# musyoku/chainer-speech-recognition

Hardware: AMD Instinct MI355X
Metric: utterances/sec (T=1000, 40x3 feat, |V|~3000) CTC train step (higher is better)
Workload: dtype bf16

## Files before the change

chainer-speech-recognition_amd/asr/_lib.py:

```python
import ctypes
import os

import torch

_HERE = os.path.dirname(os.path.abspath(__file__))
_ACT = os.environ.get("ASR_ACT", "").lower()
LIB_PATH = os.environ.get("ASR_HIP_LIB") or os.path.join(os.path.dirname(_HERE),
                                                        "libasr_hip_f16.so" if _ACT in ("f16", "fp16", "float16", "half") else "libasr_hip.so")

_lib = None


def act_dtype():
    return torch.float16 if lib().asr_act_dtype() else torch.bfloat16


def debug_flag(key, default):
    for item in os.environ.get("ASR_DEBUG", "").split(","):
        k, _, v = item.strip().partition("=")
        if k == key and v:
            return int(v)
    return default

c_void_p, c_int, c_float, c_size_t = ctypes.c_void_p, ctypes.c_int, ctypes.c_float, ctypes.c_size_t
# ... 150 lines not shown
    "asr_crelu_bwd": (c_int, [c_void_p] * 4 + [c_longlong, c_int]),
    "asr_softmax_fwd": (c_int, [c_void_p] * 3 + [c_longlong, c_int, c_int]),
    "asr_softmax_bwd": (c_int, [c_void_p] * 4 + [c_longlong, c_int, c_int]),
    "asr_avgpool_h_fwd": (c_int, [c_void_p] * 3 + [c_longlong, c_int, c_int, c_int]),
    "asr_avgpool_h_bwd": (c_int, [c_void_p] * 3 + [c_longlong, c_int, c_int, c_int]),
    "asr_unpool_h_fwd": (c_int, [c_void_p] * 3 + [c_longlong, c_int, c_int, c_int, c_int]),
    "asr_unpool_h_bwd": (c_int, [c_void_p] * 3 + [c_longlong, c_int, c_int, c_int, c_int]),
    "asr_gaussian_noise": (c_int, [c_void_p] * 3 + [c_longlong, c_float, ctypes.c_uint]),
    "asr_maxpool_h_indexes": (c_int, [c_void_p, c_void_p, c_void_p, c_longlong, c_int, c_int, c_int]),
    "asr_upsample_h_fwd": (c_int, [c_void_p] * 4 + [c_longlong] + [c_int] * 4),
    "asr_upsample_h_bwd": (c_int, [c_void_p] * 4 + [c_longlong] + [c_int] * 4),
    "asr_spp_bins": (c_int, [c_int]),
    "asr_spp_fwd": (c_int, [c_void_p] * 4 + [c_int] * 5),
    "asr_spp_bwd": (c_int, [c_void_p] * 4 + [c_int] * 5),
    "asr_sgd_ctl": (c_int, [c_void_p] * 4 + [c_longlong, c_int] + [c_float] * 3 + [c_void_p]),
}

_ERRORS = {-1: "bad argument", -2: "workspace too small", -3: "unsupported shape", -4: "kernel launch failed"}


class AsrHipError(RuntimeError):
    pass


def lib():
    global _lib
    if _lib is None:
        if not os.path.isfile(LIB_PATH):
            raise AsrHipError("%s not found: build it with `make -C %s` (hipcc, gfx950). There is no CPU fallback."
                              % (LIB_PATH, os.path.dirname(LIB_PATH)))
# ... 27 lines not shown
```

chainer-speech-recognition_amd/asr/_ops.py:

```python
import os

import torch

from . import _lib
from ._lib import check, ptr, stream

BF16 = _lib.act_dtype()
F32 = torch.float32


def _is_bf16(t):
    if t.dtype == BF16:
        return 1
    if t.dtype == F32:
        return 0
    raise TypeError("expected float32 or bfloat16, got %s" % t.dtype)


def gemm_nt(a, b, bias=None, out_dtype=BF16, out=None):
    assert a.dtype == BF16 and b.dtype == BF16 and a.dim() == 2 and b.dim() == 2
    assert a.stride(1) == 1 and b.stride(1) == 1 and a.shape[1] == b.shape[1]
    M, K = a.shape
    N = b.shape[0]
    if out is None:
# ... 528 lines not shown
def clear_abort_words(dev):
    for w in abort_words():
        if w.device == dev:
            w.zero_()


def step_control(g, partials, clip, grad_scale, alpha, beta1, beta2, applied, ctl, any_abort=None, reserved_index=-1, loss_scale=None):
    if any_abort is None:
        any_abort = gather_abort(g.device)
    rc = _lib.lib().asr_step_control_scaled(stream(), ptr(g), g.numel(), ptr(partials), ptr(any_abort), None, float(clip),
                                            float(grad_scale), float(alpha), float(beta1), float(beta2), ptr(applied), ptr(ctl),
                                            int(reserved_index), None if loss_scale is None else ptr(loss_scale))
    check(rc, "asr_step_control_scaled")


def sqnorm_partials_count(n):
    return int(_lib.lib().asr_sqnorm_partials_count(int(n)))


def adam_ctl(p, g, m, v, beta1, beta2, eps, weight_decay, ctl):
    rc = _lib.lib().asr_adam_ctl(stream(), ptr(p), ptr(g), ptr(m), ptr(v), p.numel(), beta1, beta2, eps, weight_decay, ptr(ctl))
    check(rc, "asr_adam_ctl")


def sgd_ctl(p, g, v, kind, lr, momentum, weight_decay, ctl):
    rc = _lib.lib().asr_sgd_ctl(stream(), ptr(p), ptr(g), ptr(v), p.numel(), int(kind), lr, momentum, weight_decay, ptr(ctl))
    check(rc, "asr_sgd_ctl")


SRU_CHUNKED = [True]
# ... 568 lines not shown
```

chainer-speech-recognition_amd/asr/functions.py:

```python
import math
import os

import torch

from . import _ops
from ._lib import debug_flag as _lib_debug
from .link import grad_buffer, grads_queued

BF16, F32 = _ops.BF16, torch.float32


_SIDE = {"streams": {}, "origins": {}, "enabled": True, "dirty": set(), "keep": [], "keep_bytes": 0,
         "join_before_recurrence": _lib_debug("side_join", 0) != 0}
_KEEP_LIMIT = 512
_KEEP_BYTES_LIMIT = int(_lib_debug("side_keep_gb", 48)) << 30


def side_stream():
    if not _SIDE["enabled"]:
        return None
    cur = torch.cuda.current_stream()
    key = cur.cuda_stream
    st = _SIDE["streams"].get(key)
    if st is None:
# ... 359 lines not shown


def conv_weight_matrix_bwd(W):
    return _ops.conv_weight_pack_bwd(W.contiguous())


def conv_weight_matrix_pad8(W):
    Co, Ci, KH, KW = W.shape
    Wp = torch.zeros((Co, 8, KH, KW), dtype=W.dtype, device=W.device)
    Wp[:, :Ci] = W
    return _ops.conv_weight_pack(Wp, Kp=(KH * KW * 8 + 31) // 32 * 32)


def convolution_2d(x, W, b, link, pad=(0, 0), causal=False, out_f32=False):
    pad_h, pad_t = (pad, pad) if isinstance(pad, int) else pad
    w16 = link.compute_copy("w16", W, conv_weight_matrix)
    w16t = link.compute_copy("w16t", W, conv_weight_matrix_t)
    wbwd = link.compute_copy("wbwd", W, conv_weight_matrix_bwd) if _ops.conv_implicit_ok(W.shape[0], W.shape[2], W.shape[3]) else None
    if x.dtype not in (F32, BF16):
        raise TypeError("convolution input must be float32 or bfloat16")
    w16p = link.compute_copy("w16p", W, conv_weight_matrix_pad8) if W.shape[1] < 8 else None
    y = _Conv2D.apply(x, W, b, w16, w16t, wbwd, w16p, int(pad_h), int(pad_t), bool(causal), bool(out_f32))
    return logical4(y)


def convolution_2d_given_weight(x, W, b, link, pad=(0, 0), causal=False, out_f32=False):
    pad_h, pad_t = (pad, pad) if isinstance(pad, int) else pad
    with torch.no_grad():
        w16 = conv_weight_matrix(W.detach())
        w16t = conv_weight_matrix_t(W.detach())
        wbwd = conv_weight_matrix_bwd(W.detach()) if _ops.conv_implicit_ok(W.shape[0], W.shape[2], W.shape[3]) else None
        w16p = conv_weight_matrix_pad8(W.detach()) if W.shape[1] < 8 else None
    y = _Conv2D.apply(x, W, b, w16, w16t, wbwd, w16p, int(pad_h), int(pad_t), bool(causal), bool(out_f32))
    return logical4(y)


# ... 51 lines not shown
        return False
    Co, Ci, KH, KW = wshape
    if not _ops.conv_mp_ok(Ci, KH, KW, Co, k) or Ci >= 8:
        return False
    return x.shape[2] + 2 * pad_h - KH + 1 >= 1 and (x.shape[3] if causal else x.shape[3] + 2 * pad_t - KW + 1) >= 1


def convolution_maxout_pool(x, W, b, link, pad, causal, k, given_weight=False):
    pad_h, pad_t = (pad, pad) if isinstance(pad, int) else pad
    if not convolution_maxout_pool_ok(x, tuple(W.shape), pad, causal, k):
        return None
    if given_weight:
        with torch.no_grad():
            w16q = conv_weight_matrix_pad8_128(W.detach())
    else:
        w16q = link.compute_copy("w16q", W, conv_weight_matrix_pad8_128)
    return logical4(_ConvMaxoutPool.apply(x, W, b, w16q, int(pad_h), int(pad_t), bool(causal), int(k)))


class _Dense(torch.autograd.Function):

    @staticmethod
    def forward(ctx, x2, W, b, w16, w16t, out_f32):
        y = _ops.gemm_nt(x2, w16, b.detach() if b is not None else None, F32 if out_f32 else BF16)
        ctx.save_for_backward(x2, w16t)
        ctx.params = (W, b)
        ctx.need_dx = ctx.needs_input_grad[0]
        if out_f32:
            ctx._asr_mailbox = _GradMailbox(y, b)
        return y

# ... 686 lines not shown
```

chainer-speech-recognition_amd/asr/link.py:

```python
import contextlib
import math

import torch

from . import _lib

F32 = torch.float32
BF16 = _lib.act_dtype()

_WEIGHT_EPOCH = [0]


def bump_weight_epoch():
    _WEIGHT_EPOCH[0] += 1


class Parameter(torch.nn.Parameter):

    def __new__(cls, data=None):
        if data is None:
            data = torch.empty(0, dtype=F32)
        return super().__new__(cls, data, requires_grad=True)


class Link(torch.nn.Module):
    def __init__(self):
        super().__init__()
        object.__setattr__(self, "_compute_cache", {})
        object.__setattr__(self, "_cast_registry", {})

    @contextlib.contextmanager
    def init_scope(self):
        yield

    @property
    def xp(self):
        return torch

    def params(self):
        return self.parameters()

    def namedparams(self):
        for name, p in self.named_parameters():
            yield "/" + name.replace(".", "/"), p
# ... 18 lines not shown
            if p is not None and p.numel() == 0 and src is not None and src.numel() > 0:
                p.data = torch.empty(src.shape, dtype=p.dtype, device=p.device)
        super()._load_from_state_dict(state_dict, prefix, *args, **kwargs)
        bump_weight_epoch()

    def compute_copy(self, key, param, maker, layout=None):
        stamp = (_WEIGHT_EPOCH[0], param._version, param.data_ptr())
        hit = self._compute_cache.get(key)
        if hit is not None and hit[0] == stamp:
            _await_copy(hit)
            return hit[1]
        with torch.no_grad():
            value = maker(param.detach())
        self._compute_cache[key] = _made_copy(stamp, value)
        if layout is not None and value.is_cuda:
            self._cast_registry[key] = (param, value, _cast_jobs(param, layout))
        return value


def _made_copy(stamp, value):
    if not value.is_cuda:
        return (stamp, value, None, None)
    cur = torch.cuda.current_stream()
    return (stamp, value, {"stream": cur, "event": None}, {cur.cuda_stream})


def _await_copy(entry):
    if entry[2] is None:
        return
    cur = torch.cuda.current_stream()
    if cur.cuda_stream not in entry[3]:
# ... 8 lines not shown

def _cast_jobs(param, layout):
    n, shape = param.numel(), tuple(param.shape)
    if layout == "plain":
        return ((0, 0, n // shape[-1], shape[-1], 0),)
    if layout == "t_first":
        return ((0, 0, shape[0], n // shape[0], 1),)
    if layout == "t_last":
        return ((0, 0, n // shape[-1], shape[-1], 1),)
    if layout == "t_each":
        each = shape[-2] * shape[-1]
        return tuple((i * each, i * each, shape[-2], shape[-1], 1) for i in range(n // each))
    raise ValueError(layout)


def refresh_compute_copies(model):
    from . import _lib
    todo, sig = [], []
    for m in model.modules():
        reg = getattr(m, "_cast_registry", None)
        if not reg:
            continue
        for key, (param, out, jobs) in reg.items():
            hit = m._compute_cache.get(key)
            if hit is None or hit[1] is not out or hit[0][2] != param.data_ptr() or not param.is_cuda:
                continue
            todo.append((m, key, param, out))
            sig.append((param.data_ptr(), out.data_ptr(), jobs))
    if not todo:
        return 0
    cached = getattr(model, "_cast_table", None)
    if cached is None or cached[0] != sig:
        rows, tile = [], 0
        for src, dst, jobs in sig:
            for so, do, r, c, t in jobs:
                rows.append([src + 4 * so, dst + 2 * do, r, c, t, tile])
                tile += ((r + 63) // 64) * ((c + 63) // 64)
        table = torch.tensor(rows, dtype=torch.int64).to(todo[0][2].device)
        cached = (sig, table, len(rows), tile)
        object.__setattr__(model, "_cast_table", cached)
    _lib.check(_lib.lib().asr_cast_bf16_many(_lib.stream(), _lib.ptr(cached[1]), cached[2], cached[3]), "asr_cast_bf16_many")
    for m, key, param, out in todo:
        m._compute_cache[key] = _made_copy((_WEIGHT_EPOCH[0], param._version, param.data_ptr()), out)
    return cached[2]


class Chain(Link):
    pass


_GRAD_LISTENER = [None]


def grads_queued(*params):
    if _GRAD_LISTENER[0] is not None:
        _GRAD_LISTENER[0]([p for p in params if p is not None])


def grad_buffer(param):
# ... 89 lines not shown
```

chainer-speech-recognition_amd/asr/optimizers.py:

```python
import torch

from . import _ops
from .link import bump_weight_epoch, refresh_compute_copies

F32 = torch.float32
RESERVED = 64


class GradientClipping(object):
    name = "GradientClipping"

    def __init__(self, threshold):
        self.threshold = threshold


class WeightDecay(object):
    name = "WeightDecay"

    def __init__(self, rate):
        self.rate = rate


class Optimizer(object):
    def __init__(self):
# ... 66 lines not shown
        any_abort = _ops.gather_abort(G.device, G[0:1] if self.communicator is not None else None)
        scale = 1.0
        if self.communicator is not None:
            self.communicator.finish_backward(self)
            scale = 1.0 / self.communicator.size
        self.t += 1
        clip, decay = 0.0, 0.0
        for h in self._hooks:
            if isinstance(h, GradientClipping):
                clip = float(h.threshold)
            elif isinstance(h, WeightDecay):
                decay = float(h.rate)
        alpha, beta1, beta2 = self._control_constants()
        _ops.step_control(G, self._flat["partials"], clip, scale, alpha, beta1, beta2, self._flat["applied"], self._flat["ctl"],
                          any_abort, 0, self._loss_scale_buffer(G.device))
        self._step(P, G, decay, self._flat["ctl"])
        bump_weight_epoch()
        refresh_compute_copies(self.target)
        try:
            self._raise_if_previous_step_gave_up()
        finally:
            self._watch_gave_up()

    def _watch_gave_up(self):
        st = self._gave_up
        if st[0] is None:
            st[0] = torch.zeros(1, dtype=F32).pin_memory()
        if st[1] is None or st[1].query():
            st[0].copy_(self._flat["ctl"][6:7], non_blocking=True)
            st[1] = torch.cuda.Event()
            st[1].record()
            st[2] = self.t

# ... 110 lines not shown
        self.alpha, self.beta1, self.beta2, self.eps = alpha, beta1, beta2, eps

        self.m = self.v = None

    def _init_state(self, total, dev, old):
        self.m = self._carried(total, dev, old, self.m)
        self.v = self._carried(total, dev, old, self.v)

    def _control_constants(self):
        return self.alpha, self.beta1, self.beta2

    def _state_buffers(self):
        return [self.m, self.v]

    def _step(self, P, G, decay, ctl):
        _ops.adam_ctl(P, G, self.m, self.v, self.beta1, self.beta2, self.eps, decay, ctl)


class SGD(Optimizer):
    kind = 0

    def __init__(self, lr=0.01):
        super().__init__()
        self.lr = lr
        self.momentum = 0.0
        self.vel = None

    def _init_state(self, total, dev, old):
        if self.kind:
            self.vel = self._carried(total, dev, old, self.vel)

# ... 75 lines not shown
```

chainer-speech-recognition_amd/csrc/elementwise.hip:

```cpp
#include "common.hpp"
#include "../../include/asr_hip.h"

namespace asr {
namespace ew {

constexpr int kThreads = 256;
static inline int grid_for(long long n) {
    long long g = (n + kThreads - 1) / kThreads;
    if (g > 256 * 16) g = 256 * 16;
    if (g < 1) g = 1;
    return (int)g;
}

__global__ void cast_bf16_kernel(const float* __restrict__ src, uint16_t* __restrict__ dst, long long n) {
    for (long long i = blockIdx.x * (long long)blockDim.x + threadIdx.x; i < n; i += (long long)gridDim.x * blockDim.x)
        dst[i] = f32_to_bf16(src[i]);
}
__global__ void cast_bf16_vec8_kernel(const float4* __restrict__ src, uint4* __restrict__ dst, long long n8) {
    for (long long i = blockIdx.x * (long long)blockDim.x + threadIdx.x; i < n8; i += (long long)gridDim.x * blockDim.x) {
        const float4 a = src[2 * i], b = src[2 * i + 1];
        uint4 o;
        o.x = (uint32_t)f32_to_bf16(a.x) | ((uint32_t)f32_to_bf16(a.y) << 16);
        o.y = (uint32_t)f32_to_bf16(a.z) | ((uint32_t)f32_to_bf16(a.w) << 16);
        o.z = (uint32_t)f32_to_bf16(b.x) | ((uint32_t)f32_to_bf16(b.y) << 16);
// ... 401 lines not shown
        if (transpose) dst[(long long)k * Co + co] = f32_to_bf16(v); else dst[i] = f32_to_bf16(v);
    }
}
__global__ void conv_weight_pack_bwd_kernel(const float* __restrict__ W, uint16_t* __restrict__ dst, int Co, int Ci, int KH,
                                            int KW) {
    const long long n = (long long)Co * Ci * KH * KW;
    for (long long i = blockIdx.x * (long long)blockDim.x + threadIdx.x; i < n; i += (long long)gridDim.x * blockDim.x) {
        long long r = i;
        const int co = (int)(r % Co); r /= Co;
        const int kw = (int)(r % KW); r /= KW;
        const int kh = (int)(r % KH);
        const int ci = (int)(r / KH);
        dst[i] = f32_to_bf16(W[(((long long)co * Ci + ci) * KH + kh) * KW + kw]);
    }
}
__global__ void conv_weight_grad_unpack_kernel(const float* __restrict__ scratch, float* __restrict__ gW, int Co, int Ci,
                                               int KH, int KW, int Kp, int Cs, int copies) {
    const long long n = (long long)Co * Ci * KH * KW;
    for (long long i = blockIdx.x * (long long)blockDim.x + threadIdx.x; i < n; i += (long long)gridDim.x * blockDim.x) {
        long long r = i;
        const int kw = (int)(r % KW); r /= KW;
        const int kh = (int)(r % KH); r /= KH;
        const int ci = (int)(r % Ci);
        const int co = (int)(r / Ci);
        const long long o = (long long)co * Kp + (kh * KW + kw) * Cs + ci;
        float v = scratch[o];
        for (int c = 1; c < copies; ++c) v += scratch[o + (long long)c * Co * Kp];
        gW[i] += v;
    }
}
// ... 567 lines not shown
    if (!x || !y || n <= 0 || ratio < 0.f || ratio >= 1.f) return ASR_ERR_BAD_ARG;
    hipLaunchKernelGGL(dropout_kernel, dim3(grid_for(n)), dim3(kThreads), 0, (hipStream_t)stream, (const uint16_t*)x,
                       (uint16_t*)y, n, ratio, seed);
    ASR_LAUNCH_CHECK();
    return ASR_OK;
}

extern "C" int asr_conv_weight_pack(void* stream, const float* W, void* dst, int Co, int Ci, int KH, int KW, int Kp,
                                    int transpose) {
    if (!W || !dst || Co <= 0 || Ci <= 0 || KH <= 0 || KW <= 0 || Kp < KH * KW * Ci) return ASR_ERR_BAD_ARG;
    hipLaunchKernelGGL(conv_weight_pack_kernel, dim3(grid_for((long long)Co * Kp)), dim3(kThreads), 0, (hipStream_t)stream,
                       W, (uint16_t*)dst, Co, Ci, KH, KW, Kp, transpose);
    ASR_LAUNCH_CHECK();
    return ASR_OK;
}
extern "C" int asr_conv_weight_pack_bwd(void* stream, const float* W, void* dst, int Co, int Ci, int KH, int KW) {
    if (!W || !dst || Co <= 0 || Ci <= 0 || KH <= 0 || KW <= 0) return ASR_ERR_BAD_ARG;
    hipLaunchKernelGGL(conv_weight_pack_bwd_kernel, dim3(grid_for((long long)Co * Ci * KH * KW)), dim3(kThreads), 0, (hipStream_t)stream,
                       W, (uint16_t*)dst, Co, Ci, KH, KW);
    ASR_LAUNCH_CHECK();
    return ASR_OK;
}
extern "C" int asr_conv_weight_grad_unpack_copies(void* stream, const float* scratch, int copies, float* gW, int Co, int Ci, int KH,
                                                  int KW, int Kp, int Cs) {
    if (Cs <= 0) Cs = Ci;
    if (!scratch || !gW || Co <= 0 || Ci <= 0 || KH <= 0 || KW <= 0 || Cs < Ci || Kp < KH * KW * Cs || copies < 1 || copies > 8)
        return ASR_ERR_BAD_ARG;
    hipLaunchKernelGGL(conv_weight_grad_unpack_kernel, dim3(grid_for((long long)Co * Ci * KH * KW)), dim3(kThreads), 0,
                       (hipStream_t)stream, scratch, gW, Co, Ci, KH, KW, Kp, Cs, copies);
    ASR_LAUNCH_CHECK();
// ... 27 lines not shown
```

chainer-speech-recognition_amd/csrc/optim.hip:

```cpp
#include "common.hpp"
#include "../../include/asr_hip.h"

namespace asr {
namespace optim {

__global__ __launch_bounds__(256) void sqnorm_kernel(const float* __restrict__ g, long long n, float* __restrict__ out) {
    __shared__ float scratch[32];
    float s = 0.f;
    for (long long i = blockIdx.x * (long long)blockDim.x + threadIdx.x; i < n; i += (long long)gridDim.x * blockDim.x) {
        const float v = g[i];
        s += v * v;
    }
    s = block_sum(s, scratch);
    if (threadIdx.x == 0) atomicAdd(out, s);
}

__global__ __launch_bounds__(256) void adam_kernel(float* __restrict__ p, const float* __restrict__ g,
                                                   float* __restrict__ m, float* __restrict__ v, long long n, float lr_t,
                                                   float beta1, float beta2, float eps, float decay, float clip,
                                                   float grad_scale, const float* __restrict__ sqnorm) {
    float rate = grad_scale;
    if (sqnorm) {
        if (!isfinite(sqnorm[0])) return;
        if (clip > 0.f) {
// ... 98 lines not shown
        const float r = clip / norm;
        if (r < 1.f) rate *= r;
    }
    int t = applied[0];
    if (!drop) applied[0] = ++t;
    const double tt = t < 1 ? 1.0 : (double)t;
    const double fix1 = 1.0 - pow((double)beta1, tt), fix2 = 1.0 - pow((double)beta2, tt);
    ctl[0] = drop ? 1.f : 0.f;
    ctl[1] = rate;
    ctl[2] = (float)((double)alpha * sqrt(fix2) / fix1);
    ctl[3] = (float)t;
    ctl[5] = gave_up ? 1.f : 0.f;
    if (gave_up) ctl[6] += 1.f;
}

__global__ __launch_bounds__(256) void adam_ctl_kernel(float* __restrict__ p, const float* __restrict__ g, float* __restrict__ m,
                                                       float* __restrict__ v, long long n, float beta1, float beta2, float eps,
                                                       float decay, const float* __restrict__ ctl) {
    if (ctl[0] != 0.f) return;
    const float rate = ctl[1], lr_t = ctl[2];
    for (long long i = blockIdx.x * (long long)blockDim.x + threadIdx.x; i < n; i += (long long)gridDim.x * blockDim.x) {
        const float pi = p[i];
        const float gi = g[i] * rate + decay * pi;
        float mi = m[i], vi = v[i];
        mi += (1.f - beta1) * (gi - mi);
        vi += (1.f - beta2) * (gi * gi - vi);
        m[i] = mi;
        v[i] = vi;
        p[i] = pi - lr_t * mi / (sqrtf(vi) + eps);
    }
}

__global__ __launch_bounds__(256) void sgd_ctl_kernel(float* __restrict__ p, const float* __restrict__ g, float* __restrict__ v,
                                                      long long n, int kind, float lr, float mu, float decay,
                                                      const float* __restrict__ ctl) {
    if (ctl[0] != 0.f) return;
    const float rate = ctl[1];
    for (long long i = blockIdx.x * (long long)blockDim.x + threadIdx.x; i < n; i += (long long)gridDim.x * blockDim.x) {
        const float pi = p[i];
        const float gi = g[i] * rate + decay * pi;
        if (kind == 0) {
            p[i] = pi - lr * gi;
        } else {
            const float vi = mu * v[i] - lr * gi;
// ... 81 lines not shown
                                float clip_threshold, float grad_scale, float alpha, float beta1, float beta2,
                                int* applied_steps, float* ctl, int reserved_index) {
    return asr_step_control_scaled(stream, g, n, partials, abort0, abort1, clip_threshold, grad_scale, alpha, beta1, beta2,
                                   applied_steps, ctl, reserved_index, nullptr);
}

extern "C" int asr_adam_ctl(void* stream, float* p, const float* g, float* m, float* v, long long n, float beta1, float beta2,
                            float eps, float weight_decay, const float* ctl) {
    if (!p || !g || !m || !v || !ctl || n <= 0) return ASR_ERR_BAD_ARG;
    hipLaunchKernelGGL(adam_ctl_kernel, dim3(grid_for(n)), dim3(256), 0, (hipStream_t)stream, p, g, m, v, n, beta1, beta2, eps,
                       weight_decay, ctl);
    ASR_LAUNCH_CHECK();
    return ASR_OK;
}

extern "C" int asr_sgd_ctl(void* stream, float* p, const float* g, float* v, long long n, int kind, float lr, float momentum,
                           float weight_decay, const float* ctl) {
    if (!p || !g || !ctl || n <= 0 || kind < 0 || kind > 2 || (kind > 0 && !v)) return ASR_ERR_BAD_ARG;
    hipLaunchKernelGGL(sgd_ctl_kernel, dim3(grid_for(n)), dim3(256), 0, (hipStream_t)stream, p, g, v, n, kind, lr, momentum,
                       weight_decay, ctl);
    ASR_LAUNCH_CHECK();
    return ASR_OK;
}
```

include/asr_hip.h:

```cpp
#ifndef ASR_HIP_H
#define ASR_HIP_H
#include <stddef.h>
#include <stdint.h>
#ifdef __cplusplus
extern "C" {
#endif

int asr_version(void);
int asr_act_dtype(void);
int asr_stream_delay(void* stream, int microseconds);
int asr_occupy_cus(void* stream, int microseconds, int lds_bytes, int blocks);
int asr_stream_traffic(void* stream, int microseconds, int lds_bytes, int blocks, void* buf, long long bytes);

size_t asr_ctc_workspace_bytes(int T, int B, int V, int Lmax, int gram);
int asr_ctc_forward(void* stream, const float* xs, const int32_t* label_unigram, const int32_t* label_bigram,
                    const int32_t* x_len, const int32_t* l_len, int T, int B, int V, int Lmax, int blank,
                    float* loss_per_utt, float* loss_mean, void* workspace, size_t workspace_bytes);
int asr_ctc_forward_lse(void* stream, const float* xs, const int32_t* label_unigram, const int32_t* label_bigram,
                        const int32_t* x_len, const int32_t* l_len, int T, int B, int V, int Lmax, int blank, float* loss_per_utt,
                        float* loss_mean, void* workspace, size_t workspace_bytes, const float* row_lse);
int asr_ctc_backward(void* stream, const float* xs, const int32_t* x_len, int T, int B, int V, int Lmax, int gram,
                     const float* gy, int gy_per_utt, float scale, float* grad, const void* workspace,
                     size_t workspace_bytes);
int asr_ctc_loss_grad(void* stream, const float* xs, const int32_t* label_unigram, const int32_t* label_bigram,
// ... 126 lines not shown
                       int KH, int KW, int Tr, int Hr, int N);
int asr_conv_nt_8pn(void* stream, const void* x, const void* W, int ldw, void* out, int out_bf16, const float* bias, int Ts, int B, int Hs,
                    int Cs, int KH, int KW, int pad_h, int pad_t, int sgn, int Tr, int Hr, int N);
int asr_conv_direct_ok(int Ts, int B, int Hs, int Cs, int KH, int KW, int Tr, int Hr, int N, int K, int out_bf16);
int asr_conv_direct_nt(void* stream, const void* x, const void* W, int ldw, void* out, const float* bias, int Ts, int B, int Hs, int Cs,
                       int KH, int KW, int pad_h, int pad_t, int sgn, int Tr, int Hr, int N);
int asr_conv_mp_ok(int Ci, int KH, int KW, int Co, int k);
int asr_conv_mp_fwd(void* stream, const void* x8, const void* W, int ldw, const float* bias, void* y, void* idx, int Ts, int B, int Hs,
                    int KH, int KW, int pad_h, int pad_t, int Tout, int Hout, int Co, int k);
long long asr_conv_mp_bwd_workspace(int Tout, int B, int Hout, int Co, int k);
int asr_conv_mp_bwd(void* stream, const void* gy, const void* idx, const void* x8, void* workspace, float* gW, float* gb, int Ts, int B,
                    int Hs, int Ci, int KH, int KW, int pad_h, int pad_t, int Tout, int Hout, int Co, int k);
int asr_pack_input_pad(void* stream, const void* x, int x_bf16, long long sT, long long sB, long long sH, long long sC, int T,
                       int B, int H, int C, int Cpad, void* out_bf16);
int asr_conv_weight_pack_bwd(void* stream, const float* W, void* dst, int Co, int Ci, int KH, int KW);
int asr_conv_tn_acc(void* stream, const void* g, int ldg, const void* x, float* C, int ldc, int Co, int Ts, int B, int Hs,
                    int Cs, int KH, int KW, int pad_h, int pad_t, int Tr, int Hr);
int asr_conv_tn_8ph_ok(const void* g, int ldg, const void* x, const float* C, int ldc, int Co, int Ts, int B, int Hs, int Cs, int KH, int KW,
                       int Tr, int Hr);
int asr_conv_tn_acc_8ph(void* stream, const void* g, int ldg, const void* x, float* C, int ldc, int Co, int Ts, int B, int Hs, int Cs, int KH,
                        int KW, int pad_h, int pad_t, int Tr, int Hr);
int asr_conv_weight_grad_unpack(void* stream, const float* scratch, float* gW, int Co, int Ci, int KH, int KW, int Kp, int Cs);
int asr_conv_tn_copies(int Co, int Cs, int KH, int KW);
int asr_conv_tn_acc_copies(void* stream, const void* g, int ldg, const void* x, float* C, int ldc, int copies, int Co, int Ts, int B,
                           int Hs, int Cs, int KH, int KW, int pad_h, int pad_t, int Tr, int Hr);
int asr_conv_weight_grad_unpack_copies(void* stream, const float* scratch, int copies, float* gW, int Co, int Ci, int KH, int KW, int Kp,
                                       int Cs);
int asr_maxout2_fwd(void* stream, const void* x, void* y, long long n_out);
int asr_maxout2_bwd(void* stream, const void* x, const void* dy, void* dx, long long n_out);
int asr_maxout2_pool_fwd(void* stream, const void* x, void* y, long long R, int Hin, int C, int k);
// ... 78 lines not shown
                        float grad_scale, const float* sqnorm, int step);
int asr_clip_decay_sgd(void* stream, float* p, const float* g, float* v, long long n, int kind, float lr, float momentum,
                       float weight_decay, float clip_threshold, float grad_scale, const float* sqnorm);
int asr_sqnorm_partials_count(long long n);
int asr_gather_abort(void* stream, const long long* word_ptrs, int n, int* any_word, float* poison);
int asr_step_control(void* stream, const float* g, long long n, float* partials, const int* abort0, const int* abort1,
                     float clip_threshold, float grad_scale, float alpha, float beta1, float beta2, int* applied_steps,
                     float* ctl, int reserved_index);
int asr_step_control_scaled(void* stream, const float* g, long long n, float* partials, const int* abort0, const int* abort1,
                            float clip_threshold, float grad_scale, float alpha, float beta1, float beta2, int* applied_steps,
                            float* ctl, int reserved_index, float* loss_scale);
int asr_adam_ctl(void* stream, float* p, const float* g, float* m, float* v, long long n, float beta1, float beta2, float eps,
                 float weight_decay, const float* ctl);
int asr_sgd_ctl(void* stream, float* p, const float* g, float* v, long long n, int kind, float lr, float momentum,
                float weight_decay, const float* ctl);

int asr_crelu_fwd(void* stream, const void* x, void* y, long long rows, int C);
int asr_crelu_bwd(void* stream, const void* x, const void* dy, void* dx, long long rows, int C);
int asr_softmax_fwd(void* stream, const void* x, void* y, long long rows, int C, int log_form);
int asr_softmax_bwd(void* stream, const void* y, const void* dy, void* dx, long long rows, int C, int log_form);
int asr_avgpool_h_fwd(void* stream, const void* x, void* y, long long R, int Hin, int C, int k);
int asr_avgpool_h_bwd(void* stream, const void* dy, void* dx, long long R, int Hin, int C, int k);
int asr_unpool_h_fwd(void* stream, const void* x, void* y, long long R, int Hin, int Hout, int C, int k);
int asr_unpool_h_bwd(void* stream, const void* dy, void* dx, long long R, int Hin, int Hout, int C, int k);
int asr_gaussian_noise(void* stream, const void* x, void* y, long long n, float stdv, unsigned int seed);
int asr_maxpool_h_indexes(void* stream, const void* x, void* idx_u8, long long R, int Hin, int C, int k);
int asr_upsample_h_fwd(void* stream, const void* x, const void* idx_u8, void* y, long long R, int Hin, int Hout, int C, int k);
int asr_upsample_h_bwd(void* stream, const void* dy, const void* idx_u8, void* dx, long long R, int Hin, int Hout, int C, int k);
int asr_spp_bins(int pyramid_height);
int asr_spp_fwd(void* stream, const void* x, void* y, int* pos, int T, int B, int H, int C, int pyramid_height);
// ... 7 lines not shown
```

Measured before the change: 2461.

## Fuse Adam update with bf16 compute-copy refresh and batch conv weight packing

Adds an Adam kernel driven by a per-tile job table. After each 64x64 tile of parameters is updated, it writes the bf16 (optionally transposed) compute copies straight from shared memory, so the separate cast pass no longer re-reads the fp32 weights. Conv weight packs that used to be rebuilt lazily, one launch per layer, are now refreshed in a single batched launch after the step. The cost is host-side table building and signature checks, plus a more complex refresh path that could disagree with the lazy cache if the registries go out of sync.

Result: no change. 2470, median of 6 (+0.4%).

```diff
diff --git a/chainer-speech-recognition_amd/asr/_lib.py b/chainer-speech-recognition_amd/asr/_lib.py
--- a/chainer-speech-recognition_amd/asr/_lib.py
+++ b/chainer-speech-recognition_amd/asr/_lib.py
@@ -188,6 +188,8 @@
     "asr_spp_fwd": (c_int, [c_void_p] * 4 + [c_int] * 5),
     "asr_spp_bwd": (c_int, [c_void_p] * 4 + [c_int] * 5),
     "asr_sgd_ctl": (c_int, [c_void_p] * 4 + [c_longlong, c_int] + [c_float] * 3 + [c_void_p]),
+    "asr_adam_refresh": (c_int, [c_void_p] * 6 + [c_int, c_void_p, c_longlong] + [c_float] * 4 + [c_void_p]),
+    "asr_conv_weight_pack_many": (c_int, [c_void_p, c_void_p, c_int, c_longlong]),
 }
 
 _ERRORS = {-1: "bad argument", -2: "workspace too small", -3: "unsupported shape", -4: "kernel launch failed"}
diff --git a/chainer-speech-recognition_amd/asr/_ops.py b/chainer-speech-recognition_amd/asr/_ops.py
--- a/chainer-speech-recognition_amd/asr/_ops.py
+++ b/chainer-speech-recognition_amd/asr/_ops.py
@@ -566,6 +566,12 @@
     check(rc, "asr_step_control_scaled")
 
 
+def adam_refresh(p, g, m, v, jobs, njobs, tiles, ntiles, beta1, beta2, eps, weight_decay, ctl):
+    rc = _lib.lib().asr_adam_refresh(stream(), ptr(p), ptr(g), ptr(m), ptr(v), ptr(jobs), int(njobs), ptr(tiles), int(ntiles),
+                                     beta1, beta2, eps, weight_decay, ptr(ctl))
+    check(rc, "asr_adam_refresh")
+
+
 def sqnorm_partials_count(n):
     return int(_lib.lib().asr_sqnorm_partials_count(int(n)))
 
diff --git a/chainer-speech-recognition_amd/asr/functions.py b/chainer-speech-recognition_amd/asr/functions.py
--- a/chainer-speech-recognition_amd/asr/functions.py
+++ b/chainer-speech-recognition_amd/asr/functions.py
@@ -397,12 +397,13 @@
 
 def convolution_2d(x, W, b, link, pad=(0, 0), causal=False, out_f32=False):
     pad_h, pad_t = (pad, pad) if isinstance(pad, int) else pad
-    w16 = link.compute_copy("w16", W, conv_weight_matrix)
-    w16t = link.compute_copy("w16t", W, conv_weight_matrix_t)
-    wbwd = link.compute_copy("wbwd", W, conv_weight_matrix_bwd) if _ops.conv_implicit_ok(W.shape[0], W.shape[2], W.shape[3]) else None
+    Kw = W.shape[2] * W.shape[3]
+    w16 = link.compute_copy("w16", W, conv_weight_matrix, ("pack", 0, 0, (Kw * W.shape[1] + 7) // 8 * 8))
+    w16t = link.compute_copy("w16t", W, conv_weight_matrix_t, ("pack", 1, 0, (Kw * W.shape[1] + 7) // 8 * 8))
+    wbwd = link.compute_copy("wbwd", W, conv_weight_matrix_bwd, ("pack", 2, 0, 0)) if _ops.conv_implicit_ok(W.shape[0], W.shape[2], W.shape[3]) else None
     if x.dtype not in (F32, BF16):
         raise TypeError("convolution input must be float32 or bfloat16")
-    w16p = link.compute_copy("w16p", W, conv_weight_matrix_pad8) if W.shape[1] < 8 else None
+    w16p = link.compute_copy("w16p", W, conv_weight_matrix_pad8, ("pack", 0, 8, (Kw * 8 + 31) // 32 * 32)) if W.shape[1] < 8 else None
     y = _Conv2D.apply(x, W, b, w16, w16t, wbwd, w16p, int(pad_h), int(pad_t), bool(causal), bool(out_f32))
     return logical4(y)
 
@@ -484,7 +485,7 @@
         with torch.no_grad():
             w16q = conv_weight_matrix_pad8_128(W.detach())
     else:
-        w16q = link.compute_copy("w16q", W, conv_weight_matrix_pad8_128)
+        w16q = link.compute_copy("w16q", W, conv_weight_matrix_pad8_128, ("pack", 0, 8, 128))
     return logical4(_ConvMaxoutPool.apply(x, W, b, w16q, int(pad_h), int(pad_t), bool(causal), int(k)))
 
 
diff --git a/chainer-speech-recognition_amd/asr/link.py b/chainer-speech-recognition_amd/asr/link.py
--- a/chainer-speech-recognition_amd/asr/link.py
+++ b/chainer-speech-recognition_amd/asr/link.py
@@ -28,6 +28,7 @@
         super().__init__()
         object.__setattr__(self, "_compute_cache", {})
         object.__setattr__(self, "_cast_registry", {})
+        object.__setattr__(self, "_pack_registry", {})
 
     @contextlib.contextmanager
     def init_scope(self):
@@ -76,7 +77,10 @@
             value = maker(param.detach())
         self._compute_cache[key] = _made_copy(stamp, value)
         if layout is not None and value.is_cuda:
-            self._cast_registry[key] = (param, value, _cast_jobs(param, layout))
+            if isinstance(layout, tuple):
+                self._pack_registry[key] = (param, value, layout)
+            else:
+                self._cast_registry[key] = (param, value, _cast_jobs(param, layout))
         return value
 
 
@@ -115,22 +119,28 @@
     raise ValueError(layout)
 
 
-def refresh_compute_copies(model):
-    from . import _lib
-    todo, sig = [], []
+ADAM_REFRESH = [_lib.debug_flag("adam_refresh", 1) != 0]
+PACK_MANY = [_lib.debug_flag("pack_many", 1) != 0]
+STEP_TILE, STEP_RUN, STEP_COPIES = 64, 4096, 3
+
+
+def _registered(model, registry):
+    found = []
     for m in model.modules():
-        reg = getattr(m, "_cast_registry", None)
+        reg = getattr(m, registry, None)
         if not reg:
             continue
-        for key, (param, out, jobs) in reg.items():
+        for key, (param, out, spec) in reg.items():
             hit = m._compute_cache.get(key)
             if hit is None or hit[1] is not out or hit[0][2] != param.data_ptr() or not param.is_cuda:
                 continue
-            todo.append((m, key, param, out))
-            sig.append((param.data_ptr(), out.data_ptr(), jobs))
-    if not todo:
-        return 0
-    cached = getattr(model, "_cast_table", None)
+            found.append((m, key, param, out, spec))
+    return found
+
+
+def _cast_table_of(model, todo, attr="_cast_table"):
+    sig = [(param.data_ptr(), out.data_ptr(), jobs) for _, _, param, out, jobs in todo]
+    cached = getattr(model, attr, None)
     if cached is None or cached[0] != sig:
         rows, tile = [], 0
         for src, dst, jobs in sig:
@@ -139,11 +149,115 @@
                 tile += ((r + 63) // 64) * ((c + 63) // 64)
         table = torch.tensor(rows, dtype=torch.int64).to(todo[0][2].device)
         cached = (sig, table, len(rows), tile)
-        object.__setattr__(model, "_cast_table", cached)
-    _lib.check(_lib.lib().asr_cast_bf16_many(_lib.stream(), _lib.ptr(cached[1]), cached[2], cached[3]), "asr_cast_bf16_many")
-    for m, key, param, out in todo:
+        object.__setattr__(model, attr, cached)
+    return cached
+
+
+def _pack_job(param, layout):
+    _, mode, Cp, Kp = layout
+    Co, Ci, KH, KW = param.shape
+    return (Co, Ci, Cp or Ci, KH, KW, Kp, mode, Co * Ci * KH * KW if mode == 2 else Co * Kp)
+
+
+def _refresh_packs(model):
+    todo = [t for t in _registered(model, "_pack_registry") if t[2].is_contiguous()]
+    if not todo or len(todo) > 256:
+        return []
+    sig = [(param.data_ptr(), out.data_ptr(), _pack_job(param, layout)) for _, _, param, out, layout in todo]
+    cached = getattr(model, "_pack_table", None)
+    if cached is None or cached[0] != sig:
+        rows, block = [], 0
+        for src, dst, (Co, Ci, Cp, KH, KW, Kp, mode, n) in sig:
+            rows.append([src, dst, Co, Ci, Cp, KH, KW, Kp, mode, block])
+            block += (n + 255) // 256
+        cached = (sig, torch.tensor(rows, dtype=torch.int64).to(todo[0][2].device), len(rows), block)
+        object.__setattr__(model, "_pack_table", cached)
+    _lib.check(_lib.lib().asr_conv_weight_pack_many(_lib.stream(), _lib.ptr(cached[1]), cached[2], cached[3]), "asr_conv_weight_pack_many")
+    return todo
+
+
+def refresh_compute_copies(model, done=()):
+    skip = {(id(m), key) for m, key, _, _ in done}
+    todo = [t for t in _registered(model, "_cast_registry") if (id(t[0]), t[1]) not in skip]
+    count = 0
+    if todo:
+        cached = _cast_table_of(model, todo, "_cast_left_table" if done else "_cast_table")
+        _lib.check(_lib.lib().asr_cast_bf16_many(_lib.stream(), _lib.ptr(cached[1]), cached[2], cached[3]), "asr_cast_bf16_many")
+        count = cached[2]
+    packs = _refresh_packs(model) if PACK_MANY[0] else []
+    for m, key, param, out in list(done) + [t[:4] for t in todo] + [t[:4] for t in packs]:
         m._compute_cache[key] = _made_copy((_WEIGHT_EPOCH[0], param._version, param.data_ptr()), out)
-    return cached[2]
+    return count
+
+
+def step_table(total, params):
+    jobs, tiles, left = [], [], []
+
+    def add(kind, off, rows, cols, copies):
+        n = (rows + STEP_RUN - 1) // STEP_RUN if kind == 0 else ((rows + STEP_TILE - 1) // STEP_TILE) * ((cols + STEP_TILE - 1) // STEP_TILE)
+        flat = [x for c in copies for x in c] + [0] * (2 * (STEP_COPIES - len(copies)))
+        tiles.extend((len(jobs) << 32) | i for i in range(n))
+        jobs.append([kind, off, rows, cols, len(tiles) - n, len(copies)] + flat)
+
+    cursor = 0
+    for index, (off, shape, copies) in enumerate(params):
+        numel = 1
+        for d in shape:
+            numel *= d
+        assert off >= cursor and off + numel <= total
+        view = next((cj for _, cj in copies if cj[0][4]), None)
+        take = []
+        for ci, (addr, cj) in enumerate(copies):
+            if len(take) < STEP_COPIES and (not cj[0][4] or cj == view):
+                take.append((addr, cj))
+            else:
+                left.append((index, ci))
+        if not take or numel == 0:
+            continue
+        if view is None:
+            view = ((0, 0, numel // shape[-1], shape[-1], 0),)
+        if off > cursor:
+            add(0, cursor, off - cursor, 1, [])
+        covered = 0
+        for so, do, r, c, _ in view:
+            assert so == covered
+            add(1, off + so, r, c, [(addr + 2 * (do if cj[0][4] else so), 1 if cj[0][4] else 0) for addr, cj in take])
+            covered += r * c
+        assert covered == numel
+        cursor = off + numel
+    if total > cursor:
+        add(0, cursor, total - cursor, 1, [])
+    assert len(tiles) < 2 ** 31
+    return jobs, tiles, left
+
+
+def adam_refresh_plan(model, flat):
+    where = {pid: (o, n) for pid, o, n in zip(flat["ids"], flat["offsets"], flat["numels"])}
+    base = flat["P"].data_ptr()
+    by_param, order = {}, []
+    for m, key, param, out, jobs in _registered(model, "_cast_registry"):
+        at = where.get(id(param))
+        if at is None or at[1] != param.numel() or param.data_ptr() != base + 4 * at[0]:
+            continue
+        if id(param) not in by_param:
+            by_param[id(param)] = (at[0], tuple(param.shape), [])
+            order.append(id(param))
+        by_param[id(param)][2].append((m, key, param, out, jobs))
+    if not order:
+        return None
+    order.sort(key=lambda pid: by_param[pid][0])
+    sig = (base, flat["P"].numel(), tuple((by_param[pid][0], by_param[pid][1], tuple((c[3].data_ptr(), c[4]) for c in by_param[pid][2]))
+                                         for pid in order))
+    cached = getattr(model, "_step_table", None)
+    if cached is None or cached[0] != sig:
+        jobs, tiles, left = step_table(sig[1], [(o, shape, list(copies)) for o, shape, copies in sig[2]])
+        dev = flat["P"].device
+        skip = set(left)
+        done = [by_param[pid][2][ci][:4] for pi, pid in enumerate(order) for ci in range(len(by_param[pid][2])) if (pi, ci) not in skip]
+        cached = (sig, torch.tensor(jobs, dtype=torch.int64).to(dev), len(jobs), torch.tensor(tiles, dtype=torch.int64).to(dev), len(tiles), done)
+        object.__setattr__(model, "_step_table", cached)
+        _cast_table_of(model, _registered(model, "_cast_registry"))
+    return cached[1:]
 
 
 class Chain(Link):
diff --git a/chainer-speech-recognition_amd/asr/optimizers.py b/chainer-speech-recognition_amd/asr/optimizers.py
--- a/chainer-speech-recognition_amd/asr/optimizers.py
+++ b/chainer-speech-recognition_amd/asr/optimizers.py
@@ -1,6 +1,7 @@
 import torch
 
 from . import _ops
+from . import link
 from .link import bump_weight_epoch, refresh_compute_copies
 
 F32 = torch.float32
@@ -104,9 +105,9 @@
         alpha, beta1, beta2 = self._control_constants()
         _ops.step_control(G, self._flat["partials"], clip, scale, alpha, beta1, beta2, self._flat["applied"], self._flat["ctl"],
                           any_abort, 0, self._loss_scale_buffer(G.device))
-        self._step(P, G, decay, self._flat["ctl"])
+        done = self._step(P, G, decay, self._flat["ctl"]) or ()
         bump_weight_epoch()
-        refresh_compute_copies(self.target)
+        refresh_compute_copies(self.target, done)
         try:
             self._raise_if_previous_step_gave_up()
         finally:
@@ -247,7 +248,12 @@
         return [self.m, self.v]
 
     def _step(self, P, G, decay, ctl):
-        _ops.adam_ctl(P, G, self.m, self.v, self.beta1, self.beta2, self.eps, decay, ctl)
+        plan = link.adam_refresh_plan(self.target, self._flat) if link.ADAM_REFRESH[0] else None
+        if plan is None:
+            _ops.adam_ctl(P, G, self.m, self.v, self.beta1, self.beta2, self.eps, decay, ctl)
+            return ()
+        _ops.adam_refresh(P, G, self.m, self.v, plan[0], plan[1], plan[2], plan[3], self.beta1, self.beta2, self.eps, decay, ctl)
+        return plan[4]
 
 
 class SGD(Optimizer):
diff --git a/chainer-speech-recognition_amd/csrc/elementwise.hip b/chainer-speech-recognition_amd/csrc/elementwise.hip
--- a/chainer-speech-recognition_amd/csrc/elementwise.hip
+++ b/chainer-speech-recognition_amd/csrc/elementwise.hip
@@ -439,6 +439,37 @@
         dst[i] = f32_to_bf16(W[(((long long)co * Ci + ci) * KH + kh) * KW + kw]);
     }
 }
+__global__ void __launch_bounds__(256) conv_weight_pack_many_kernel(const long long* __restrict__ jobs, int njobs) {
+    __shared__ long long first_block[256];
+    if ((int)threadIdx.x < njobs) first_block[threadIdx.x] = jobs[threadIdx.x * 10 + 9];
+    __syncthreads();
+    int j = 0;
+    while (j + 1 < njobs && first_block[j + 1] <= (long long)blockIdx.x) ++j;
+    const long long* __restrict__ J = jobs + j * 10;
+    const float* __restrict__ W = (const float*)J[0];
+    uint16_t* __restrict__ dst = (uint16_t*)J[1];
+    const int Co = (int)J[2], Ci = (int)J[3], Cp = (int)J[4], KH = (int)J[5], KW = (int)J[6], Kp = (int)J[7], mode = (int)J[8];
+    const long long i = ((long long)blockIdx.x - first_block[j]) * 256 + threadIdx.x;
+    if (mode == 2) {
+        if (i >= (long long)Co * Ci * KH * KW) return;
+        long long r = i;
+        const int co = (int)(r % Co); r /= Co;
+        const int kw = (int)(r % KW); r /= KW;
+        const int kh = (int)(r % KH);
+        const int ci = (int)(r / KH);
+        dst[i] = f32_to_bf16(W[(((long long)co * Ci + ci) * KH + kh) * KW + kw]);
+        return;
+    }
+    if (i >= (long long)Co * Kp) return;
+    const int K = KH * KW * Cp;
+    const int co = (int)(i / Kp), k = (int)(i - (long long)co * Kp);
+    float v = 0.f;
+    if (k < K) {
+        const int ci = k % Cp, kw = (k / Cp) % KW, kh = k / (Cp * KW);
+        if (ci < Ci) v = W[(((long long)co * Ci + ci) * KH + kh) * KW + kw];
+    }
+    if (mode == 1) dst[(long long)k * Co + co] = f32_to_bf16(v); else dst[i] = f32_to_bf16(v);
+}
 __global__ void conv_weight_grad_unpack_kernel(const float* __restrict__ scratch, float* __restrict__ gW, int Co, int Ci,
                                                int KH, int KW, int Kp, int Cs, int copies) {
     const long long n = (long long)Co * Ci * KH * KW;
@@ -1036,6 +1067,13 @@
     ASR_LAUNCH_CHECK();
     return ASR_OK;
 }
+extern "C" int asr_conv_weight_pack_many(void* stream, const long long* jobs_dev, int njobs, long long total_blocks) {
+    if (!jobs_dev || njobs <= 0 || njobs > 256 || total_blocks <= 0 || total_blocks > 0x7fffffffLL) return ASR_ERR_BAD_ARG;
+    hipLaunchKernelGGL(conv_weight_pack_many_kernel, dim3((unsigned)total_blocks), dim3(256), 0, (hipStream_t)stream, jobs_dev, njobs);
+    ASR_LAUNCH_CHECK();
+    return ASR_OK;
+}
+
 extern "C" int asr_conv_weight_pack_bwd(void* stream, const float* W, void* dst, int Co, int Ci, int KH, int KW) {
     if (!W || !dst || Co <= 0 || Ci <= 0 || KH <= 0 || KW <= 0) return ASR_ERR_BAD_ARG;
     hipLaunchKernelGGL(conv_weight_pack_bwd_kernel, dim3(grid_for((long long)Co * Ci * KH * KW)), dim3(kThreads), 0, (hipStream_t)stream,
diff --git a/chainer-speech-recognition_amd/csrc/optim.hip b/chainer-speech-recognition_amd/csrc/optim.hip
--- a/chainer-speech-recognition_amd/csrc/optim.hip
+++ b/chainer-speech-recognition_amd/csrc/optim.hip
@@ -136,20 +136,128 @@
     if (gave_up) ctl[6] += 1.f;
 }
 
+__device__ __forceinline__ float rounded(float x) {
+    asm("" : "+v"(x));
+    return x;
+}
+__device__ __forceinline__ void adam_elem(float& pi, float graw, float& mi, float& vi, float rate, float decay, float beta1,
+                                          float beta2, float eps, float lr_t) {
+    const float gi = rounded(graw * rate) + rounded(decay * pi);
+    mi = mi + rounded((1.f - beta1) * (gi - mi));
+    vi = __builtin_fmaf(1.f - beta2, __builtin_fmaf(gi, gi, -vi), vi);
+    pi = pi - rounded(lr_t * mi) / (sqrtf(vi) + eps);
+}
+
 __global__ __launch_bounds__(256) void adam_ctl_kernel(float* __restrict__ p, const float* __restrict__ g, float* __restrict__ m,
                                                        float* __restrict__ v, long long n, float beta1, float beta2, float eps,
                                                        float decay, const float* __restrict__ ctl) {
     if (ctl[0] != 0.f) return;
     const float rate = ctl[1], lr_t = ctl[2];
     for (long long i = blockIdx.x * (long long)blockDim.x + threadIdx.x; i < n; i += (long long)gridDim.x * blockDim.x) {
-        const float pi = p[i];
-        const float gi = g[i] * rate + decay * pi;
-        float mi = m[i], vi = v[i];
-        mi += (1.f - beta1) * (gi - mi);
-        vi += (1.f - beta2) * (gi * gi - vi);
+        float pi = p[i], mi = m[i], vi = v[i];
+        adam_elem(pi, g[i], mi, vi, rate, decay, beta1, beta2, eps, lr_t);
         m[i] = mi;
         v[i] = vi;
-        p[i] = pi - lr_t * mi / (sqrtf(vi) + eps);
+        p[i] = pi;
+    }
+}
+
+constexpr int kJobWords = 12;
+__global__ __launch_bounds__(256) void adam_refresh_kernel(float* __restrict__ p, const float* __restrict__ g, float* __restrict__ m,
+                                                           float* __restrict__ v, const long long* __restrict__ jobs,
+                                                           const long long* __restrict__ tiles, float beta1, float beta2, float eps,
+                                                           float decay, const float* __restrict__ ctl) {
+    __shared__ float tile[64][65];
+    if (ctl[0] != 0.f) return;
+    const float rate = ctl[1], lr_t = ctl[2];
+    const long long which = tiles[blockIdx.x];
+    const long long* __restrict__ J = jobs + (which >> 32) * kJobWords;
+    const int local = (int)(which & 0x7fffffffLL);
+    const long long off = J[1];
+    if (J[0] == 0) {
+        const long long len = J[2];
+        const bool vec = (off & 3) == 0;
+        for (int pass = 0; pass < 4; ++pass) {
+            const long long i = (long long)local * 4096 + pass * 1024 + threadIdx.x * 4;
+            if (i >= len) break;
+            const long long e = off + i;
+            if (vec && i + 4 <= len) {
+                float4 pp = *(const float4*)(p + e), mm = *(const float4*)(m + e), vv = *(const float4*)(v + e);
+                const float4 gg = *(const float4*)(g + e);
+                adam_elem(pp.x, gg.x, mm.x, vv.x, rate, decay, beta1, beta2, eps, lr_t);
+                adam_elem(pp.y, gg.y, mm.y, vv.y, rate, decay, beta1, beta2, eps, lr_t);
+                adam_elem(pp.z, gg.z, mm.z, vv.z, rate, decay, beta1, beta2, eps, lr_t);
+                adam_elem(pp.w, gg.w, mm.w, vv.w, rate, decay, beta1, beta2, eps, lr_t);
+                *(float4*)(m + e) = mm; *(float4*)(v + e) = vv; *(float4*)(p + e) = pp;
+            } else {
+                for (int k = 0; k < 4 && i + k < len; ++k) {
+                    float pi = p[e + k], mi = m[e + k], vi = v[e + k];
+                    adam_elem(pi, g[e + k], mi, vi, rate, decay, beta1, beta2, eps, lr_t);
+                    m[e + k] = mi; v[e + k] = vi; p[e + k] = pi;
+                }
+            }
+        }
+        return;
+    }
+    const int rows = (int)J[2], cols = (int)J[3], ncopies = (int)J[5];
+    const int tiles_c = (cols + 63) / 64;
+    const int r0 = (local / tiles_c) * 64, c0 = (local % tiles_c) * 64;
+    const int tx = threadIdx.x & 15, ty = threadIdx.x >> 4;
+    const bool vec = (cols & 3) == 0 && (off & 3) == 0;
+    for (int i = ty; i < 64; i += 16) {
+        const int r = r0 + i, c = c0 + tx * 4;
+        if (r >= rows || c >= cols) continue;
+        const long long e = off + (long long)r * cols + c;
+        if (vec) {
+            float4 pp = *(const float4*)(p + e), mm = *(const float4*)(m + e), vv = *(const float4*)(v + e);
+            const float4 gg = *(const float4*)(g + e);
+            adam_elem(pp.x, gg.x, mm.x, vv.x, rate, decay, beta1, beta2, eps, lr_t);
+            adam_elem(pp.y, gg.y, mm.y, vv.y, rate, decay, beta1, beta2, eps, lr_t);
+            adam_elem(pp.z, gg.z, mm.z, vv.z, rate, decay, beta1, beta2, eps, lr_t);
+            adam_elem(pp.w, gg.w, mm.w, vv.w, rate, decay, beta1, beta2, eps, lr_t);
+            *(float4*)(m + e) = mm; *(float4*)(v + e) = vv; *(float4*)(p + e) = pp;
+            tile[i][tx * 4 + 0] = pp.x; tile[i][tx * 4 + 1] = pp.y; tile[i][tx * 4 + 2] = pp.z; tile[i][tx * 4 + 3] = pp.w;
+        } else {
+            for (int k = 0; k < 4 && c + k < cols; ++k) {
+                float pi = p[e + k], mi = m[e + k], vi = v[e + k];
+                adam_elem(pi, g[e + k], mi, vi, rate, decay, beta1, beta2, eps, lr_t);
+                m[e + k] = mi; v[e + k] = vi; p[e + k] = pi;
+                tile[i][tx * 4 + k] = pi;
+            }
+        }
+    }
+    if (ncopies == 0) return;
+    __syncthreads();
+    const bool vecc = (cols & 3) == 0, vecr = (rows & 3) == 0;
+    for (int q = 0; q < ncopies; ++q) {
+        uint16_t* __restrict__ dst = (uint16_t*)J[6 + 2 * q];
+        if (J[7 + 2 * q] == 0) {
+            for (int i = ty; i < 64; i += 16) {
+                const int r = r0 + i, c = c0 + tx * 4;
+                if (r >= rows || c >= cols) continue;
+                if (vecc) {
+                    uint2 o;
+                    o.x = (unsigned)f32_to_bf16(tile[i][tx * 4 + 0]) | ((unsigned)f32_to_bf16(tile[i][tx * 4 + 1]) << 16);
+                    o.y = (unsigned)f32_to_bf16(tile[i][tx * 4 + 2]) | ((unsigned)f32_to_bf16(tile[i][tx * 4 + 3]) << 16);
+                    *(uint2*)(dst + (size_t)r * cols + c) = o;
+                } else {
+                    for (int k = 0; k < 4 && c + k < cols; ++k) dst[(size_t)r * cols + c + k] = f32_to_bf16(tile[i][tx * 4 + k]);
+                }
+            }
+        } else {
+            for (int i = ty; i < 64; i += 16) {
+                const int c = c0 + i, r = r0 + tx * 4;
+                if (c >= cols || r >= rows) continue;
+                if (vecr) {
+                    uint2 o;
+                    o.x = (unsigned)f32_to_bf16(tile[tx * 4 + 0][i]) | ((unsigned)f32_to_bf16(tile[tx * 4 + 1][i]) << 16);
+                    o.y = (unsigned)f32_to_bf16(tile[tx * 4 + 2][i]) | ((unsigned)f32_to_bf16(tile[tx * 4 + 3][i]) << 16);
+                    *(uint2*)(dst + (size_t)c * rows + r) = o;
+                } else {
+                    for (int k = 0; k < 4 && r + k < rows; ++k) dst[(size_t)c * rows + r + k] = f32_to_bf16(tile[tx * 4 + k][i]);
+                }
+            }
+        }
     }
 }
 
@@ -261,6 +369,17 @@
     return ASR_OK;
 }
 
+extern "C" int asr_adam_refresh(void* stream, float* p, const float* g, float* m, float* v, const long long* jobs_dev, int njobs,
+                                const long long* tiles_dev, long long ntiles, float beta1, float beta2, float eps, float weight_decay,
+                                const float* ctl) {
+    if (!p || !g || !m || !v || !ctl || !jobs_dev || !tiles_dev || njobs <= 0 || ntiles <= 0 || ntiles > 0x7fffffffLL)
+        return ASR_ERR_BAD_ARG;
+    hipLaunchKernelGGL(adam_refresh_kernel, dim3((unsigned)ntiles), dim3(256), 0, (hipStream_t)stream, p, g, m, v, jobs_dev, tiles_dev,
+                       beta1, beta2, eps, weight_decay, ctl);
+    ASR_LAUNCH_CHECK();
+    return ASR_OK;
+}
+
 extern "C" int asr_sgd_ctl(void* stream, float* p, const float* g, float* v, long long n, int kind, float lr, float momentum,
                            float weight_decay, const float* ctl) {
     if (!p || !g || !ctl || n <= 0 || kind < 0 || kind > 2 || (kind > 0 && !v)) return ASR_ERR_BAD_ARG;
diff --git a/include/asr_hip.h b/include/asr_hip.h
--- a/include/asr_hip.h
+++ b/include/asr_hip.h
@@ -164,6 +164,7 @@
 int asr_pack_input_pad(void* stream, const void* x, int x_bf16, long long sT, long long sB, long long sH, long long sC, int T,
                        int B, int H, int C, int Cpad, void* out_bf16);
 int asr_conv_weight_pack_bwd(void* stream, const float* W, void* dst, int Co, int Ci, int KH, int KW);
+int asr_conv_weight_pack_many(void* stream, const long long* jobs_dev, int njobs, long long total_blocks);
 int asr_conv_tn_acc(void* stream, const void* g, int ldg, const void* x, float* C, int ldc, int Co, int Ts, int B, int Hs,
                     int Cs, int KH, int KW, int pad_h, int pad_t, int Tr, int Hr);
 int asr_conv_tn_8ph_ok(const void* g, int ldg, const void* x, const float* C, int ldc, int Co, int Ts, int B, int Hs, int Cs, int KH, int KW,
@@ -272,6 +273,9 @@
                  float weight_decay, const float* ctl);
 int asr_sgd_ctl(void* stream, float* p, const float* g, float* v, long long n, int kind, float lr, float momentum,
                 float weight_decay, const float* ctl);
+int asr_adam_refresh(void* stream, float* p, const float* g, float* m, float* v, const long long* jobs_dev, int njobs,
+                     const long long* tiles_dev, long long ntiles, float beta1, float beta2, float eps, float weight_decay,
+                     const float* ctl);
 
 int asr_crelu_fwd(void* stream, const void* x, void* y, long long rows, int C);
 int asr_crelu_bwd(void* stream, const void* x, const void* dy, void* dx, long long rows, int C);
```
